# neuraloperator/pde-policylearning

Hardware: AMD Instinct MI355X
Metric: FNO2d fwd+bwd fields/sec (higher is better)
Workload: dtype f32

## Files before the change

### include/fnoengine.h

```cpp
#ifndef FNOENGINE_H
#define FNOENGINE_H
#include <stddef.h>
#ifdef __cplusplus
extern "C" {
#endif

#define FNO_MAX_LAYERS 16
#define FNO_VERSION 100

enum { FNO_OK = 0, FNO_EINVAL = -1, FNO_EUNSUPPORTED = -2, FNO_EHIP = -3, FNO_ENOMEM = -4 };
enum { FNO_NORM_BACKWARD = 0, FNO_NORM_FORWARD = 1, FNO_NORM_ORTHO = 2 };

int fno_version(void);
const char* fno_last_error(void);
void fno_set_gemm_mode(int split_precision);
int fno_get_gemm_mode(void);
void fno_set_mode_gemm(int mfma);
int fno_get_mode_gemm(void);

void fno_set_fused_mid(int on);
int fno_get_fused_mid(void);

typedef struct FnoSpecDesc {
  int ndim;
  int Cin, Cout;
  int dims[3];
  int modes[3];
  int weight_last_extent;
  int norm;
  int input_gelu;
  int weight_planes;
} FnoSpecDesc;

typedef struct FnoSpecPlan FnoSpecPlan;
int fno_spec_plan_create(const FnoSpecDesc* desc, FnoSpecPlan** out);
void fno_spec_plan_destroy(FnoSpecPlan* plan);
size_t fno_spec_workspace_bytes(const FnoSpecPlan* plan, int batch);
size_t fno_spec_xhat_bytes(const FnoSpecPlan* plan, int batch);
int fno_spec_forward(const FnoSpecPlan* plan, int batch, const float* x, const float* const* w_corners,
                     const float* bias , float* y, float* xhat_save, void* ws, size_t ws_bytes,
                     void* stream);
int fno_spec_backward(const FnoSpecPlan* plan, int batch, const float* dy, const float* xhat_save,
                      const float* const* w_corners, float* dx, float* const* dw_corners, float* dbias, void* ws,
                      size_t ws_bytes, void* stream);

typedef struct FnoModelDesc {
  int ndim;
  int Cin, C, Cout;
  int hidden_proj;
  int n_layers;
  int dims[3];
  int modes[3];
  int norm;
  unsigned gelu_mask;
// ... 284 lines not shown
```

### pde_policylearning_amd/csrc/fno_abi.hip

```cpp
#include <hip/hip_runtime.h>

#include <cmath>
#include <cstdarg>
#include <cstdio>
#include <cstdlib>
#include <cstring>
#include <map>
#include <mutex>
#include <string>
#include <vector>

#include "../../include/fnoengine.h"
#include "fno_debug.h"
#include "k_block_bwd.h"
#include "k_block_bwd2.h"
#include "k_chanflow.h"
#include "k_chanflow_step.h"
#include "k_control_loop.h"
#include "k_action_opt.h"
#include "k_policy_opt.h"
#include "k_ns2d.h"
#include "k_pointwise.h"
#include "k_block_fwd2.h"
#include "k_block_fwd3.h"
// ... 388 lines not shown
  }
  if (rc != FNO_AXIS_GENERIC) return rc;
  if (n_out > 65535) return fail(FNO_EUNSUPPORTED, "axis pass grid too large (%d)", n_out);
  return LV(truncating ? "k_axis_generic(truncating)" : "k_axis_generic(extending)", 0, 0), launch("k_axis_generic", k_axis_generic, dim3((inner + 255) / 256, n_out, outer), dim3(256), 0, st, in, out,
                tw, n_in, n_out, inner, truncating ? 1 : 0);
}

static int lead_forward(hipStream_t st, const Geom& g, const Tables& t, bool grad_dir, int B, int C, const float* x1,
                        float* tmp, float* hat) {
  const float2* tw0 = grad_dir ? t.tw_fwd_si[0] : t.tw_fwd_sf[0];
  if (g.nlead == 1) return axis_pass(st, true, x1, hat, tw0, B, g.dims[0], g.Klead[0], g.Klast * C);
  LAUNCHCHK(axis_pass(st, true, x1, tmp, t.tw_fwd_sf[1], B * g.dims[0], g.dims[1], g.Klead[1], g.Klast * C));
  return axis_pass(st, true, tmp, hat, tw0, B, g.dims[0], g.Klead[0], g.Klead[1] * g.Klast * C);
}
static int lead_inverse(hipStream_t st, const Geom& g, const Tables& t, int B, int C, const float* hat, float* tmp,
                        float* z) {
  if (g.nlead == 1) return axis_pass(st, false, hat, z, t.tw_inv[0], B, g.Klead[0], g.dims[0], g.Klast * C);
  LAUNCHCHK(axis_pass(st, false, hat, tmp, t.tw_inv[0], B, g.Klead[0], g.dims[0], g.Klead[1] * g.Klast * C));
  return axis_pass(st, false, tmp, z, t.tw_inv[1], B * g.dims[0], g.Klead[1], g.dims[1], g.Klast * C);
}

static int g_fused_mid = getenv("FNO_NO_FUSED_MID") ? 0 : 1;
extern "C" void fno_set_fused_mid(int on) { g_fused_mid = on ? 1 : 0; }
extern "C" int fno_get_fused_mid(void) { return g_fused_mid; }
static bool fused_mid_shape_ok(const Geom& g, int C) {
  if (g.nlead != 1 || (C != 32 && C != 64) || (g.Klast * C) % 64 != 0) return false;
  if (g.dims[0] > 512) return false;
  const int nk = g.Klead[0];
  return nk == 4 || nk == 8 || nk == 12 || nk == 16;
}
static bool fused_mid_ok(const Geom& g, int C) { return g_fused_mid && fused_mid_shape_ok(g, C); }
template <int NK>
static int spec_mid_t(hipStream_t st, int C, const float2* x1, float2* hat, const float2* wm, float2* z, const float2* twT,
                      const float2* twi, int n, int inner, int K2, int conj_w, int samples, int Bm, size_t w_ms) {
  const size_t lds = (size_t)10 * NK * 64 * 8;
  const dim3 grid(inner / 64, samples), blk(64, 8);
  if (C == 32) return launch("k_spec_mid", k_spec_mid<NK, 32>, grid, blk, lds, st, x1, hat, wm, z, twT, twi, n, inner, K2, conj_w, Bm, w_ms);
  return launch("k_spec_mid", k_spec_mid<NK, 64>, grid, blk, lds, st, x1, hat, wm, z, twT, twi, n, inner, K2, conj_w, Bm, w_ms);
}
static int spectral_mid_fused(hipStream_t st, const Geom& g, const Tables& t, bool grad_dir, int samples, int C,
                              const float* x1, float* hat, const float* wm, float* z, int conj_w, int Bm = 1 << 30,
                              size_t w_ms = 0) {
  if (samples > 65535) return fail(FNO_EUNSUPPORTED, "spectral middle grid too large (%d)", samples);
  const float2* twT = grad_dir ? t.tw_fwd_si[0] : t.tw_fwd_sf[0];
  const float2 *xx = (const float2*)x1, *ww = (const float2*)wm;
  float2 *hh = (float2*)hat, *zz = (float2*)z;
  const int n = g.dims[0], inner = g.Klast * C;
  switch (g.Klead[0]) {
    case 4: return spec_mid_t<4>(st, C, xx, hh, ww, zz, twT, t.tw_inv[0], n, inner, g.Klast, conj_w, samples, Bm, w_ms / 2);
    case 8: return spec_mid_t<8>(st, C, xx, hh, ww, zz, twT, t.tw_inv[0], n, inner, g.Klast, conj_w, samples, Bm, w_ms / 2);
    case 12: return spec_mid_t<12>(st, C, xx, hh, ww, zz, twT, t.tw_inv[0], n, inner, g.Klast, conj_w, samples, Bm, w_ms / 2);
    case 16: return spec_mid_t<16>(st, C, xx, hh, ww, zz, twT, t.tw_inv[0], n, inner, g.Klast, conj_w, samples, Bm, w_ms / 2);
  }
  return fail(FNO_EUNSUPPORTED, "fused spectral middle: %d kept leading modes", g.Klead[0]);
}

static bool mode_gemm_members_ok(int Cin, int Cout) {
  return g_mode_mfma && Cin == Cout && (Cin == 32 || Cin == 64);
}
static int mode_gemm(hipStream_t st, const float* x, const float* w, float* out, int B, int Ktot, int Cin, int Cout,
                     int conj_w, int nm = 1, size_t x_ms = 0, size_t w_ms = 0, size_t o_ms = 0, int trans_w = 0) {
  if (Cout > 256) return fail(FNO_EUNSUPPORTED, "channels > 256");
  if (trans_w && !mode_gemm_members_ok(Cin, Cout)) return fail(FNO_EUNSUPPORTED, "transposed-weight contraction needs the matrix-core kernels");
  if (g_mode_mfma && nm == 1 && B <= 4 && Cin <= 64 && Cout <= 64 && (long)Ktot * Cin * Cout >= (1L << 21)) {
    const float2 *xx = (const float2*)x, *ww = (const float2*)w;
    float2* oo = (float2*)out;
    if (!trans_w) {
      const dim3 grid((Ktot + 3) / 4), blk(256);
      switch (B) {
        case 1: return LV("k_mode_gemv<1>", 0, 0), launch("k_mode_gemv", k_mode_gemv<1>, grid, blk, 0, st, xx, ww, oo, Ktot, Cin, Cout, conj_w);
        case 2: return LV("k_mode_gemv<2>", 0, 0), launch("k_mode_gemv", k_mode_gemv<2>, grid, blk, 0, st, xx, ww, oo, Ktot, Cin, Cout, conj_w);
        case 3: return LV("k_mode_gemv<3>", 0, 0), launch("k_mode_gemv", k_mode_gemv<3>, grid, blk, 0, st, xx, ww, oo, Ktot, Cin, Cout, conj_w);
        default: return LV("k_mode_gemv<4>", 0, 0), launch("k_mode_gemv", k_mode_gemv<4>, grid, blk, 0, st, xx, ww, oo, Ktot, Cin, Cout, conj_w);
      }
    } else if (conj_w) {
      const dim3 grid(Ktot), blk(256);
      const size_t lds = (size_t)Cout * (Cin + 1) * 8;
      switch (B) {
        case 1: return LV("k_mode_gemv_t<1>", 0, 0), launch("k_mode_gemv_t", k_mode_gemv_t<1>, grid, blk, lds, st, xx, ww, oo, Ktot, Cout, Cin);
        case 2: return LV("k_mode_gemv_t<2>", 0, 0), launch("k_mode_gemv_t", k_mode_gemv_t<2>, grid, blk, lds, st, xx, ww, oo, Ktot, Cout, Cin);
        case 3: return LV("k_mode_gemv_t<3>", 0, 0), launch("k_mode_gemv_t", k_mode_gemv_t<3>, grid, blk, lds, st, xx, ww, oo, Ktot, Cout, Cin);
        default: return LV("k_mode_gemv_t<4>", 0, 0), launch("k_mode_gemv_t", k_mode_gemv_t<4>, grid, blk, lds, st, xx, ww, oo, Ktot, Cout, Cin);
      }
    }
  }
// ... 673 lines not shown
template <typename CP, typename P>
static CP corner_ptrs(const Geom& g, P spec_w, int lo, int hi) {
  CP cp;
  memset(&cp, 0, sizeof(cp));
  for (int l = lo; l <= hi; ++l)
    for (int c = 0; c < (1 << g.nlead); ++c) cp.p[l - lo][c] = (std::remove_reference_t<decltype(cp.p[0][0])>)spec_w[l][c];
  return cp;
}

template <int CIN, int COUT>
static int launch_pw(const FnoModelPlan* p, hipStream_t st, int grid, const PwFwdArgs& a, const char* name) {
  const size_t lds = pw_fwd_lds_bytes(CIN, COUT, p->NPX, a.W, a.K2in, a.NJ, a.z != nullptr, a.x1 != nullptr);
  if (p->NPX == 128)
    return GT(1), launch(name, k_pw_fwd<CIN, COUT, 128>, dim3(grid), dim3((COUT / 32) * 4 * 64), lds, st, a);
  return GT(1), launch(name, k_pw_fwd<CIN, COUT, 256>, dim3(grid), dim3((COUT / 32) * 8 * 64), lds, st, a);
}
static int launch_lift(const FnoModelPlan* p, hipStream_t st, int grid, const PwFwdArgs& a) {
  const int C = p->d.C;
  switch (p->d.Cin * 100 + C) {
    case 132: return launch_pw<1, 32>(p, st, grid, a, "k_pw_fwd_lift");
    case 232: return launch_pw<2, 32>(p, st, grid, a, "k_pw_fwd_lift");
    case 332: return launch_pw<3, 32>(p, st, grid, a, "k_pw_fwd_lift");
    case 432: return launch_pw<4, 32>(p, st, grid, a, "k_pw_fwd_lift");
    case 164: return launch_pw<1, 64>(p, st, grid, a, "k_pw_fwd_lift");
    case 264: return launch_pw<2, 64>(p, st, grid, a, "k_pw_fwd_lift");
    case 364: return launch_pw<3, 64>(p, st, grid, a, "k_pw_fwd_lift");
    case 464: return launch_pw<4, 64>(p, st, grid, a, "k_pw_fwd_lift");
  }
  return fail(FNO_EUNSUPPORTED, "lifting %d -> %d", p->d.Cin, C);
}
static bool lift_fused(const FnoModelPlan* p) {
  return p->d.Cin > 0 && g_gemm_x3 && p->NPX == 128 && !p->loose;
}
template <int C>
static bool blk_fwd_t_ok(const FnoModelPlan* p, const PwFwdArgs& a, size_t* lds) {
  if (p->NPX != 128 || p->loose || !a.x) return false;
  if ((size_t)a.PW * 4 * C >= (size_t)1 << 31) return false;
  if (a.z && a.K2in > 8) return false;
  if (C == 32) return false;
  *lds = blk_fwd_t_lds_bytes(C, a.W, a.K2in, a.NJ, a.z != nullptr, a.x1 != nullptr);
  return *lds + 2048 <= FNO_LDS_MAX;
}
static const int g_bfwd_v2 = getenv("FNO_BFWD_V2") ? 1 : 0;
static const int g_zigzag = getenv("FNO_NO_ZIGZAG") ? 0 : 1;
static bool blk_fwd_s_ok(const FnoModelPlan* p, const PwFwdArgs& a, size_t* lds) {
  if (g_bfwd_v2 || p->NPX != 128 || p->loose || !a.x || !a.u || !a.z || !a.xmax) return false;
  if (a.W != 128 || a.K2in < 1 || a.K2in > 8 || a.relu_out || a.add || (a.lw && a.CL > 4)) return false;
  if (a.x1 && (a.NJ != 1 || a.K2out > 8)) return false;
  if ((size_t)a.PW * 4 * 64 >= (size_t)1 << 31) return false;
  *lds = blk_fwd_s_lds_bytes(a.K2out, a.x1 != nullptr);
  return *lds <= FNO_LDS_MAX;
}
template <bool ACT_IN, bool LIFT>
static int launch_blk_fwd_s(const char* nm, hipStream_t st, dim3 grid, size_t lds, int epi, const PwFwdArgs& a) {
  if (epi == 2) return launch(nm, k_blk_fwd_s<ACT_IN, 2, LIFT>, grid, dim3(256), lds, st, a);
  if (epi == 1) return launch(nm, k_blk_fwd_s<ACT_IN, 1, LIFT>, grid, dim3(256), lds, st, a);
  return launch(nm, k_blk_fwd_s<ACT_IN, 0, LIFT>, grid, dim3(256), lds, st, a);
}
template <int C>
static int launch_block_x3(const FnoModelPlan* p, hipStream_t st, int grid, const PwFwdArgs& a, bool* ub_published = nullptr) {
  bool unused = false;
  bool& published = ub_published ? *ub_published : unused;
  published = false;
  const bool lift_ub = a.lw && a.ubound && a.xmax;
  const char* nm = a.lw ? "k_pw_fwd_block0" : "k_pw_fwd_block";
  size_t lds_t = 0, lds_s = 0;
// ... 146 lines not shown
template <int C>
static int launch_pfwd_c(const FnoModelPlan* p, hipStream_t st, int grid, const ProjFwdArgs& a) {
  return a.CO == 1 ? launch_pfwd_cn<C, 1>(p, st, grid, a) : launch_pfwd_cn<C, PROJ_MAXCO>(p, st, grid, a);
}
template <int C, int NCO>
static int launch_pbwd_cn(const FnoModelPlan* p, hipStream_t st, int grid, const ProjBwdArgs& a) {
  const size_t lds = proj_bwd_lds_bytes(C, kHID, p->NPX, NCO);
  GT(1);
  if (p->NPX == 128) return launch("k_proj_bwd", k_proj_bwd<C, kHID, 128, NCO>, dim3(grid), dim3(512), lds, st, a);
  return launch("k_proj_bwd", k_proj_bwd<C, kHID, 256, NCO>, dim3(grid), dim3(1024), lds, st, a);
}
static bool use_pbwd_t(int C, int CO, int npx) {
  return g_gemm_x3 && (C == 64 || C == 32) && CO == 1 && npx == 128;
}
static int w1_frag_items(int HID, int C) { return (HID / 32) * (C / 16) * 64 + (HID / 32) * 2 * (C / 32) * 64; }
static int pack_w1_x3(hipStream_t st, const float* w1, unsigned short* wa1, unsigned short* wa3, int HID, int C) {
  return launch("k_pack_w1_x3", k_pack_w1_t<3>, dim3((w1_frag_items(HID, C) + 255) / 256), dim3(256), 0, st, w1, wa1, wa3, HID, C,
                (const float*)nullptr);
}
template <int C>
static int launch_pbwd_c(const FnoModelPlan* p, hipStream_t st, int grid, const ProjBwdArgs& a) {
  const size_t lds_t = proj_bwd_t_lds_bytes(C, a);
  if (a.wa1 && use_pbwd_t(C, a.CO, p->NPX)) {
    if (a.amax) return GT(2), launch("k_proj_bwd", k_proj_bwd_t<C, kHID, false, 2>, dim3(grid), dim3(512), lds_t, st, a);
    if (lds_t <= FNO_LDS_MAX) return GT(3), launch("k_proj_bwd", k_proj_bwd_t<C, kHID, false>, dim3(grid), dim3(512), lds_t, st, a);
  }
  return a.CO == 1 ? launch_pbwd_cn<C, 1>(p, st, grid, a) : launch_pbwd_cn<C, PROJ_MAXCO>(p, st, grid, a);
}
static int blk_fwd_grid(const FnoModelPlan* p, int ntiles) {
  return std::min(ntiles, (g_gemm_x3 ? FNO_GRID_PWX : FNO_GRID_PW) * p->ncu);
}

static int spectral_mid_fwd(const FnoModelPlan* p, hipStream_t st, int B, const ModelWs& w, const float* wp,
                            float* hat) {
  const Geom& g = p->g;
  const int C = p->d.C;
  if (fused_mid_ok(g, C)) return spectral_mid_fused(st, g, p->t, false, B, C, w.x1, hat, wp, w.z, 0);
  LAUNCHCHK(lead_forward(st, g, p->t, false, B, C, w.x1, w.tmp, hat));
  LAUNCHCHK(mode_gemm(st, hat, wp, w.ohat, B, g.Ktot, C, C, 0));
  return lead_inverse(st, g, p->t, B, C, w.ohat, w.tmp, w.z);
}
static int spectral_mid_adj(const FnoModelPlan* p, hipStream_t st, const ModelSizes& s, int B, int nm, const float* x1, float* tmp,
                            float* ohat, const float* xhat, float* dwp, const float* wps, const float* wpts, float* hat, float* z) {
  const Geom& g = p->g;
  const int C = p->d.C;
  const bool adj_mfma = mode_gemm_members_ok(C, C);
  const size_t hs = nm > 1 ? s.n_hat : 0, ws = nm > 1 ? s.n_wp : 0;
  LAUNCHCHK(lead_forward(st, g, p->t, true, nm * B, C, x1, tmp, ohat));
  if (dwp) LAUNCHCHK(mode_gemm_dw(st, xhat, ohat, dwp, B, g.Ktot, C, C, nm, 0, hs, ws));
  LAUNCHCHK(mode_gemm(st, ohat, adj_mfma ? wps : wpts, hat, B, g.Ktot, C, C, 1, nm, hs, ws, hs, adj_mfma ? 1 : 0));
  return lead_inverse(st, g, p->t, nm * B, C, hat, tmp, z);
}

static int tail_check(const FnoModelPlan* p, const FnoBlockTail* t, bool backward) {
  if (!t) return FNO_OK;
  const FnoModelDesc& d = p->d;
  if (d.Cin != 0 || d.Cout != 0 || d.n_layers != 1) return fail(FNO_EUNSUPPORTED, "block tail: one-layer block stacks only");
  if (p->NPX != 128 || p->loose || !row_fast_ok(p->g, d.C))
    return fail(FNO_EUNSUPPORTED, "block tail: 32 / 64 channels, rows of 32 / 64 / 128 floats");
  if (t->drop_p < 0.f || t->drop_p >= 1.f) return fail(FNO_EINVAL, "block tail: dropout rate %g outside [0, 1)", (double)t->drop_p);
  if (t->drop_p > 0.f && !t->drop_seed) return fail(FNO_EINVAL, "block tail: dropout needs the two seed words (device pointer)");
  if (backward && t->relu_out && !t->y) return fail(FNO_EINVAL, "block tail: the backward of a ReLU tail needs the forward's output");
  return FNO_OK;
}
static int model_forward_impl(const FnoModelPlan* p, int B, const FnoModelParams* prm, const float* x, float* y,
                              void* saved, void* ws, size_t ws_bytes, void* stream, const FnoBlockTail* tail);
extern "C" int fno_model_forward(const FnoModelPlan* p, int B, const FnoModelParams* prm, const float* x, float* y,
                                 void* saved, void* ws, size_t ws_bytes, void* stream) {
  return model_forward_impl(p, B, prm, x, y, saved, ws, ws_bytes, stream, nullptr);
}
extern "C" int fno_model_forward_tail(const FnoModelPlan* p, int B, const FnoModelParams* prm, const float* x, float* y,
                                      void* saved, void* ws, size_t ws_bytes, void* stream, const FnoBlockTail* tail) {
  if (!tail) return fail(FNO_EINVAL, "fno_model_forward_tail: null tail");
  return model_forward_impl(p, B, prm, x, y, saved, ws, ws_bytes, stream, tail);
}
static int model_forward_impl(const FnoModelPlan* p, int B, const FnoModelParams* prm, const float* x, float* y,
                              void* saved, void* ws, size_t ws_bytes, void* stream, const FnoBlockTail* tail) {
  if (!p || !prm || !x || !y || B < 1) return fail(FNO_EINVAL, "fno_model_forward: bad argument");
  if (!saved) return fail(FNO_EINVAL, "fno_model_forward: `saved` buffer required (fno_model_saved_bytes)");
  LAUNCHCHK(tail_check(p, tail, false));
  hipStream_t st = (hipStream_t)stream;
  const Geom& g = p->g;
  const FnoModelDesc& d = p->d;
  const int C = d.C, L = d.n_layers;
  const ModelSizes s = model_sizes(p, B);
  bool ok;
  ModelWs w = carve_model(p, B, ws, ws_bytes, false, &ok);
  if (!ok) return fail(FNO_ENOMEM, "workspace too small: need %zu, have %zu", w.total, ws_bytes);
  const ModelSaved sv = carve_saved(p, B, saved);
  float* const u = sv.u;
  float* const amax = sv.bounds;
  const bool h2 = g_gemm_x3 && d.Cout > 0 && (size_t)B * g.PW >= ((size_t)1 << 17);
  static_assert(kNAmax == 64, "k_pack_w_tiled clears 64 slots");
  LAUNCHCHK(pack_w_layers(st, g, C, C, corner_ptrs<CornerPtrsL>(g, prm->spec_w, 0, L - 1), L, sv.wps,
                          mode_gemm_members_ok(C, C) && !fused_mid_shape_ok(g, C) ? nullptr : sv.wpts, s.n_wp, h2 ? amax : nullptr));

  const bool has_lift = d.Cin > 0, has_proj = d.Cout > 0;
  bool lift_xmax = false;
  bool u0_bound = false;
  FnoModelPlan::CallState cs;
  cs.B = B;
  PwFwdArgs a;
  if (has_lift) {
    memset(&a, 0, sizeof(a));
    a.x = x; a.w = prm->lift_w; a.bias = prm->lift_b;
    cs.u0_skipped = lift_fused(p);
    a.u = cs.u0_skipped ? nullptr : u; a.x1 = p->loose ? nullptr : w.x1; a.tfwd = p->t.tfwd_f;
    set_tile_geom(a, g, s, 0);
    const size_t lds_lr = ((size_t)2 * g.Klast * (g.W + 4) + (size_t)LR_ROWS * d.Cin * (g.W + 4) + 2) * 4 + (size_t)LR_ROWS * g.Klast * (d.Cin + 1) * 8;
    if (cs.u0_skipped && !p->loose && lds_lr <= 48 * 1024) {
      const int nrows = B * g.P;
      LAUNCHCHK(launch("k_lift_rowdft", k_lift_rowdft, dim3((nrows + LR_ROWS - 1) / LR_ROWS), dim3(256), lds_lr, st, x,
                       prm->lift_w, prm->lift_b, p->t.tfwd_f, (float2*)w.x1, d.Cin, C, g.PW, g.W, g.P, g.Klast, nrows,
                       h2 ? amax + kBndX : nullptr));
      lift_xmax = h2;
    } else
    LAUNCHCHK(launch_lift(p, st, std::min(s.ntiles, FNO_GRID_LIFT * p->ncu), a));
    if (p->loose) LAUNCHCHK(row_forward(st, g, p->t.tfwd_f, p->t.tT[0], p->t.K2P, B, C, u, w.x1));
  } else if (tail && tail->drop_p > 0.f) {
    RowMod mod;
    mod.drop_seed = tail->drop_seed; mod.drop_p = tail->drop_p;
    LAUNCHCHK(row_forward(st, g, p->t.tfwd_f, p->t.tT[0], p->t.K2P, B, C, x, w.x1, 0, &mod));
  } else {
    LAUNCHCHK(row_forward(st, g, p->t.tfwd_f, p->t.tT[0], p->t.K2P, B, C, x, w.x1));
  }

  for (int l = 0; l < L; ++l) {
    if (p->loose && l > 0)
      LAUNCHCHK(row_forward(st, g, p->t.tfwd_f, p->t.tT[0], p->t.K2P, B, C, u + (size_t)l * s.n_act, w.x1,
                            (int)((d.gelu_mask >> (l - 1)) & 1u)));
    LAUNCHCHK(spectral_mid_fwd(p, st, B, w, sv.wps + (size_t)l * s.n_wp, sv.hats + (size_t)l * s.n_hat));
    memset(&a, 0, sizeof(a));
    a.x = (l == 0 && !has_lift) ? x : u + (size_t)l * s.n_act;
    if (l == 0 && has_lift && cs.u0_skipped) { a.x = x; a.lw = prm->lift_w; a.lb = prm->lift_b; a.CL = d.Cin; }
    a.w = prm->skip_w[l];
    a.bias = prm->spec_bias ? prm->spec_bias + (size_t)l * C : nullptr;
    a.z = w.z; a.tinv = p->t.tinv_f;
    a.u = (l == L - 1 && !has_proj) ? y : u + (size_t)(l + 1) * s.n_act;
    a.x1 = (l + 1 < L && !p->loose) ? w.x1 : nullptr;
    a.tfwd = p->t.tfwd_f;
    set_tile_geom(a, g, s, g.Klast);
    a.act_in = (l > 0) && ((d.gelu_mask >> (l - 1)) & 1u);
    a.act_out = (d.gelu_mask >> l) & 1u;
    a.relu_out = tail && tail->relu_out;
    if (h2) {
      a.umax = amax + bnd_u(l + 1);
      if (l == 0) { a.xmax = (a.lw && lift_xmax) ? amax + kBndX : nullptr; a.ubound = amax + bnd_u(0); }
      else a.xmax = amax + bnd_u(l);
    }
    a.rev = g_zigzag ? (l & 1) : 0;
    bool ub = false;
    LAUNCHCHK(launch_block(p, st, blk_fwd_grid(p, s.ntiles), a, &ub));
    if (l == 0) u0_bound = ub;
  }

  if (!has_proj) { p->put_call(saved, cs); return FNO_OK; }
  ProjFwdArgs pa;
  memset(&pa, 0, sizeof(pa));
  pa.x = u + (size_t)L * s.n_act; pa.w1 = prm->proj_w1; pa.b1 = prm->proj_b1; pa.w2 = prm->proj_w2; pa.b2 = prm->proj_b2;
  pa.y = y; pa.PW = g.PW; pa.CO = d.Cout; pa.act_in = (d.gelu_mask >> (L - 1)) & 1u;
  pa.tiles_per_plane = g.PW / 128; pa.ntiles = B * pa.tiles_per_plane;
  pa.xmax = h2 ? amax + bnd_u(L) : nullptr;
  cs.h2_fwd = h2;
  cs.bwd_clean = h2;
// ... 1933 lines not shown
```

### pde_policylearning_amd/csrc/k_pointwise.h

```cpp
#pragma once
#include "fno_dev.h"

static constexpr int FNO_OCC_PW = 4;
static constexpr int FNO_OCC_PWX = 2;

struct PwFwdArgs {
  const float* x;
  const float* w;
  const float* bias;
  const float* z;
  const float* tinv;
  float* u;
  float* x1;
  const float* tfwd;
  const float* add;
  int PW, W, P, K2in, K2out, NJ;
  int act_in, act_out;
  int relu_out;
  int loose;
  const float* lw;
  const float* lb;
  int CL;
  int tiles_per_plane, ntiles;
  const float* xmax;
// ... 340 lines not shown
#pragma unroll
            for (int h8 = 0; h8 < 2; ++h8) {
              float t[8];
#pragma unroll
              for (int j = 0; j < 8; ++j) t[j] = acc[q][8 * h8 + j];
              gelu8(t, six, inf);
#pragma unroll
              for (int j = 0; j < 8; ++j) xp[((j & 3) + 8 * (2 * h8 + (j >> 2))) * PITCH] = t[j];
            }
          } else {
#pragma unroll
            for (int r = 0; r < 16; ++r) xp[((r & 3) + 8 * (r >> 2)) * PITCH] = acc[q][r];
          }
        }
      }
      if (a.umax) absmax_publish(vmax, a.umax);
    }
    FNO_STAMP(tslot + 5);
    if (a.x1) {
      __syncthreads();
      FNO_STAMP(tslot + 6);
      row_dft_epilogue<C, NPX, NW>(xs, tfwd_s, a.W + 4, a.x1, b, px0, a.P, a.W, a.K2out, a.NJ, wave, lane);
    }
    FNO_STAMP(tslot + 7);
    __syncthreads();
    tslot += 8;
  }
}

constexpr int LR_ROWS = 8;
__global__ void __launch_bounds__(256) k_lift_rowdft(const float* __restrict__ x, const float* __restrict__ lw,
                                                     const float* __restrict__ lb, const float* __restrict__ tfwd,
                                                     float2* __restrict__ x1, int CL, int C, int PW, int W, int P, int K2,
                                                     int nrows, float* __restrict__ xmax) {
  extern __shared__ __attribute__((aligned(16))) float smem[];
  const int WP = W + 4;
  float* ts = smem;
  float* xs = ts + 2 * K2 * WP;
  float2* xh = reinterpret_cast<float2*>(xs + ((LR_ROWS * CL * WP + 1) & ~1));
  const int tid = threadIdx.x, lane = tid & 63, wave = tid >> 6;
  const int row0 = blockIdx.x * LR_ROWS;
  const int nr = min(LR_ROWS, nrows - row0);
  float vmax = 0.f;
  const int c = lane;
  float wv[4];
#pragma unroll
  for (int k = 0; k < 4; ++k) wv[k] = (c < C && k < CL) ? lw[c * CL + k] : 0.f;
  const float bc = (lb && c < C) ? lb[c] : 0.f;
  {
    const int nt_tab = 2 * K2 * W, nt_x = LR_ROWS * CL * W;
    for (int base = 0; base < nt_tab; base += 8 * 256) {
      float v[8];
#pragma unroll
      for (int q = 0; q < 8; ++q) { const int i = base + q * 256 + tid; v[q] = i < nt_tab ? tfwd[i] : 0.f; }
#pragma unroll
      for (int q = 0; q < 8; ++q) { const int i = base + q * 256 + tid; if (i < nt_tab) ts[(i / W) * WP + i % W] = v[q]; }
    }
    for (int base = 0; base < nt_x; base += 8 * 256) {
      float v[8];
#pragma unroll
      for (int q = 0; q < 8; ++q) {
        const int i = base + q * 256 + tid;
        const int rk = i / W, w = i - rk * W, r = rk / CL, k = rk - r * CL;
        const int row = row0 + r;
        const int b = row / P, prow = row - b * P;
        v[q] = (i < nt_x && r < nr) ? x[((size_t)b * CL + k) * PW + (size_t)prow * W + w] : 0.f;
      }
#pragma unroll
      for (int q = 0; q < 8; ++q) {
        const int i = base + q * 256 + tid;
        if (i < nt_x) { xs[(i / W) * WP + i % W] = v[q]; vmax = fmaxf(vmax, fabsf(v[q])); }
      }
    }
  }
  if (xmax) {
#pragma unroll
    for (int o = 32; o >= 1; o >>= 1) vmax = fmaxf(vmax, __shfl_xor(vmax, o, 64));
    __shared__ float wmax[4];
    if (lane == 0) wmax[wave] = vmax;
    __syncthreads();
    vmax = fmaxf(fmaxf(wmax[0], wmax[1]), fmaxf(wmax[2], wmax[3]));
    if (wave == 0 && (blockIdx.x & 15) == 0) absmax_publish(vmax, xmax);
  }
  __syncthreads();
  for (int i = tid; i < LR_ROWS * K2 * (CL + 1); i += 256) {
    const int r = i / (K2 * (CL + 1)), k2 = (i / (CL + 1)) % K2, k = i % (CL + 1);
    const float* tr = ts + (2 * k2) * WP;
    const float* ti = tr + WP;
    float sr = 0.f, si = 0.f;
    if (k < CL) {
      const float* xr = xs + (r * CL + k) * WP;
      float sr2 = 0.f, si2 = 0.f;
#pragma unroll 4
      for (int w = 0; w < W; w += 4) {
        const float4 xv = *reinterpret_cast<const float4*>(xr + w), tv = *reinterpret_cast<const float4*>(tr + w),
                     uv = *reinterpret_cast<const float4*>(ti + w);
        sr = fmaf(xv.x, tv.x, sr); si = fmaf(xv.x, uv.x, si);
        sr2 = fmaf(xv.y, tv.y, sr2); si2 = fmaf(xv.y, uv.y, si2);
        sr = fmaf(xv.z, tv.z, sr); si = fmaf(xv.z, uv.z, si);
        sr2 = fmaf(xv.w, tv.w, sr2); si2 = fmaf(xv.w, uv.w, si2);
      }
      sr += sr2; si += si2;
    } else {
      for (int w = 0; w < W; ++w) { sr += tr[w]; si += ti[w]; }
    }
    xh[i] = make_float2(sr, si);
  }
  __syncthreads();
  if (c < C) {
    float2* dst = x1 + (size_t)row0 * K2 * C + c;
    for (int p = wave; p < nr * K2; p += 4) {
      const float2* h = xh + p * (CL + 1);
      float sr = bc * h[CL].x, si = bc * h[CL].y;
#pragma unroll
      for (int k = 0; k < 4; ++k)
        if (k < CL) { sr = fmaf(wv[k], h[k].x, sr); si = fmaf(wv[k], h[k].y, si); }
      dst[(size_t)p * C] = make_float2(sr, si);
    }
  }
  if (xmax && wave == 0 && (blockIdx.x & 15) != 0) absmax_publish(vmax, xmax);
}
```

### pde_policylearning_amd/csrc/k_spectral_mid.h

```cpp
#pragma once
#include "fno_dev.h"

template <int NR, int SEGS = 8, bool TLDS = false>
__global__ void __launch_bounds__(64 * SEGS) k_axis_fwd(const float2* __restrict__ in, float2* __restrict__ out,
                                                        const float2* __restrict__ twT_g, int n_in, int inner) {
  extern __shared__ __attribute__((aligned(16))) float smem[];
  float2* sh = reinterpret_cast<float2*>(smem);
  const int ql = threadIdx.x;
  const int seg = __builtin_amdgcn_readfirstlane(threadIdx.y);
  const int q = blockIdx.x * 64 + ql;
  const int o = blockIdx.y;
  const float2* twT = twT_g;
  if constexpr (TLDS) {
    for (int i = threadIdx.y * 64 + threadIdx.x; i < n_in * NR; i += 64 * SEGS) sh[i] = twT_g[i];
    __syncthreads();
    twT = sh;
  }
  float2 acc[NR];
#pragma unroll
  for (int r = 0; r < NR; ++r) acc[r] = make_float2(0.f, 0.f);
  if (q < inner) {
    const float2* src = in + (size_t)o * n_in * inner + q;
    for (int nb = seg; nb < n_in; nb += 8 * SEGS) {
      float2 v[8];
// ... 978 lines not shown
      const size_t b = e / PW, p = e % PW;
      s += dy[(b * C + c) * PW + p];
    }
  }
  for (int off = 32; off > 0; off >>= 1) s += __shfl_xor(s, off, 64);
  __shared__ float sh[4];
  if ((threadIdx.x & 63) == 0) sh[threadIdx.x >> 6] = s;
  __syncthreads();
  if (threadIdx.x == 0) part[(size_t)blockIdx.x * C + c] = sh[0] + sh[1] + sh[2] + sh[3];
}

#ifdef FNO_TRACE
#define MID_STAMP(slot) do { if (blockIdx.x == 2 && blockIdx.y == gridDim.y / 2 && threadIdx.x == 0) \
    g_trace[threadIdx.y * 256 + (slot)] = __builtin_readcyclecounter(); \
    if (blockIdx.x == 0 && threadIdx.x == 0 && threadIdx.y == 0 && ((slot) == 0 || (slot) == 7)) \
    g_trace[8 * 256 + blockIdx.y * 2 + ((slot) == 7)] = __builtin_readcyclecounter(); \
    if (blockIdx.x == 1 && threadIdx.x == 0 && threadIdx.y == 0 && blockIdx.y < 64)  \
    g_trace[10 * 256 + blockIdx.y * 8 + (slot)] = __builtin_readcyclecounter(); } while (0)
#else
#define MID_STAMP(slot) do { } while (0)
#endif
template <bool B> struct MidFlag { static constexpr bool value = B; };
template <bool SREG>
FNO_DEV void cfma_uniform(f32x2& acc, float2 w, f32x2 v, f32x2 vs) {
  if constexpr (SREG) {
    const f32x2 wp = {w.x, w.y};
    asm("v_pk_fma_f32 %0, %1, %2, %0 op_sel_hi:[0,1,1]" : "+v"(acc) : "s"(wp), "v"(v));
    asm("v_pk_fma_f32 %0, %1, %2, %0 op_sel:[1,0,0] op_sel_hi:[1,1,1]" : "+v"(acc) : "s"(wp), "v"(vs));
  } else {
    acc[0] = fmaf(w.x, v[0], acc[0]); acc[0] = fmaf(w.y, vs[0], acc[0]);
    acc[1] = fmaf(w.x, v[1], acc[1]); acc[1] = fmaf(w.y, vs[1], acc[1]);
  }
}
template <int NK, int C>
__global__ void __launch_bounds__(512, 4) k_spec_mid(const float2* __restrict__ x1, float2* __restrict__ hat,
                                                     const float2* __restrict__ wm, float2* __restrict__ z,
                                                     const float2* __restrict__ twT, const float2* __restrict__ twi, int n,
                                                     int inner, int K2, int conj_w, int Bm, size_t w_ms) {
  static_assert(C == 32 || C == 64, "whole bins per workgroup");
  constexpr bool SREG = NK <= 12;
  constexpr int SEGS = 8, JW = C / SEGS, NTH = 64 * SEGS;
  constexpr int RB = 2, NG = NK / RB;
  static_assert(NK % RB == 0, "mode groups");
  extern __shared__ __attribute__((aligned(16))) float smem[];
  float2* sh = reinterpret_cast<float2*>(smem);
  float2* ys = sh + SEGS * NK * 64;
  float2* os = ys + NK * 64;
  const int ql = threadIdx.x;
  const int seg = __builtin_amdgcn_readfirstlane(threadIdx.y);
  const int tid = seg * 64 + ql;
  const int q = blockIdx.x * 64 + ql;
  const int o = blockIdx.y;
  const int k2 = q / C, ch = q - k2 * C, lb = (ql / C) * C;
  const float2* wb = wm + (size_t)(o / Bm) * w_ms + ((size_t)k2 * C + seg * JW) * C + ch;
  MID_STAMP(0);
  if constexpr (!SREG) for (int i = tid; i < n * NK; i += NTH) sh[i] = twT[i];
  float2 wv[2][RB][JW];
  auto load_w = [&](int g, int buf) {
#pragma unroll
    for (int rr = 0; rr < RB; ++rr)
#pragma unroll
      for (int j = 0; j < JW; ++j) wv[buf][rr][j] = wb[((size_t)(g * RB + rr) * K2 * C + j) * C];
  };
  load_w(0, 0);
  {
    f32x2 acc[NK];
#pragma unroll
    for (int r = 0; r < NK; ++r) acc[r] = f32x2{0.f, 0.f};
    const float2* src = x1 + (size_t)o * n * inner + q;
    constexpr int NBR = 16;
    bool first = true;
    for (int nb = seg; nb < n; nb += NBR * SEGS) {
      float2 v[NBR];
#pragma unroll
      for (int j = 0; j < NBR; ++j) {
        const int nn = nb + SEGS * j;
        v[j] = nn < n ? src[(size_t)nn * inner] : make_float2(0.f, 0.f);
      }
      if constexpr (SREG) {
      (void)first;
      auto rows = [&](auto guard) {
        constexpr bool GUARD = decltype(guard)::value;
        float2 tw[2][NK];
#pragma unroll
        for (int r = 0; r < NK; ++r) tw[0][r] = twT[(size_t)min(nb, n - 1) * NK + r];
#pragma unroll
        for (int j = 0; j < NBR; ++j) {
          const int nn = nb + SEGS * j;
          if (j + 1 < NBR) {
#pragma unroll
            for (int r = 0; r < NK; ++r) tw[(j + 1) & 1][r] = twT[(size_t)(GUARD ? min(nn + SEGS, n - 1) : nn + SEGS) * NK + r];
          }
          if (!GUARD || nn < n) {
            const f32x2 vv = {v[j].x, v[j].y}, vs = natural_pair(-v[j].y, v[j].x);
#pragma unroll
            for (int r = 0; r < NK; ++r) cfma_uniform<true>(acc[r], tw[j & 1][r], vv, vs);
          }
        }
      };
      if (nb + SEGS * (NBR - 1) < n) rows(MidFlag<false>{}); else rows(MidFlag<true>{});
      } else {
      if (first) { __syncthreads(); first = false; }
#pragma unroll
      for (int j = 0; j < NBR; ++j) {
        const int nn = nb + SEGS * j;
        if (nn < n) {
          const float2* t = sh + nn * NK;
          const f32x2 vv = {v[j].x, v[j].y}, vs = natural_pair(-v[j].y, v[j].x);
#pragma unroll
          for (int r = 0; r < NK; ++r) cfma_uniform<false>(acc[r], t[r], vv, vs);
        }
      }
      }
    }
    if constexpr (!SREG) { if (first) __syncthreads(); }
    MID_STAMP(1);
    if constexpr (!SREG) __syncthreads();
#pragma unroll
    for (int r = 0; r < NK; ++r) sh[(seg * NK + r) * 64 + ql] = make_float2(acc[r][0], acc[r][1]);
  }
  __syncthreads();
  MID_STAMP(2);
  for (int r = seg; r < NK; r += SEGS) {
    float sx = 0.f, sy = 0.f;
#pragma unroll
    for (int k = 0; k < SEGS; ++k) { sx += sh[(k * NK + r) * 64 + ql].x; sy += sh[(k * NK + r) * 64 + ql].y; }
    ys[r * 64 + ql] = make_float2(sx, sy);
    if (hat) hat[((size_t)o * NK + r) * inner + q] = make_float2(sx, sy);
  }
  __syncthreads();
  MID_STAMP(3);
  {
    const float sg = conj_w ? -1.f : 1.f;
#pragma unroll
    for (int g = 0; g < NG; ++g) {
      if (g + 1 < NG) load_w(g + 1, (g + 1) & 1);
#pragma unroll
      for (int rr = 0; rr < RB; ++rr) {
        float ax = 0.f, ay = 0.f;
#pragma unroll
        for (int j = 0; j < JW; ++j) {
          const float2 y = ys[(g * RB + rr) * 64 + lb + seg * JW + j];
          const float2 w = wv[g & 1][rr][j];
          const float wy = sg * w.y;
          ax = fmaf(y.x, w.x, ax); ax = fmaf(-y.y, wy, ax);
          ay = fmaf(y.x, wy, ay); ay = fmaf(y.y, w.x, ay);
        }
        sh[(seg * NK + g * RB + rr) * 64 + ql] = make_float2(ax, ay);
      }
    }
  }
  MID_STAMP(4);
  __syncthreads();
  MID_STAMP(5);
  for (int r = seg; r < NK; r += SEGS) {
    float sx = 0.f, sy = 0.f;
#pragma unroll
    for (int k = 0; k < SEGS; ++k) { sx += sh[(k * NK + r) * 64 + ql].x; sy += sh[(k * NK + r) * 64 + ql].y; }
    os[r * 64 + ql] = make_float2(sx, sy);
  }
  __syncthreads();
// ... 53 lines not shown
```

Measured before the change: 30190.

## Apply lifting in mode space so first spectral layer reads raw-channel row spectra

When the lift is fused with the row DFT, the row-DFT kernel now writes row spectra of the few raw input channels (plus a constant-row spectrum for the bias) rather than of the full lifted C-channel field. The first-layer spectral middle kernel gets a LIFTIN variant that runs the column DFT on these narrow spectra and applies the linear lift and bias in mode space before the channel mixing. Because the DFT is linear, this cuts the first layer's x1 write and read from C channels down to at most four. It adds a kernel specialisation with its own lane layout that relies on the mode and channel limits holding.

```diff
diff --git a/include/fnoengine.h b/include/fnoengine.h
--- a/include/fnoengine.h
+++ b/include/fnoengine.h
@@ -20,6 +20,8 @@
 
 void fno_set_fused_mid(int on);
 int fno_get_fused_mid(void);
+void fno_set_lift_modespace(int on);
+int fno_get_lift_modespace(void);
 
 typedef struct FnoSpecDesc {
   int ndim;
diff --git a/pde_policylearning_amd/csrc/fno_abi.hip b/pde_policylearning_amd/csrc/fno_abi.hip
--- a/pde_policylearning_amd/csrc/fno_abi.hip
+++ b/pde_policylearning_amd/csrc/fno_abi.hip
@@ -444,25 +444,32 @@
 static bool fused_mid_ok(const Geom& g, int C) { return g_fused_mid && fused_mid_shape_ok(g, C); }
 template <int NK>
 static int spec_mid_t(hipStream_t st, int C, const float2* x1, float2* hat, const float2* wm, float2* z, const float2* twT,
-                      const float2* twi, int n, int inner, int K2, int conj_w, int samples, int Bm, size_t w_ms) {
+                      const float2* twi, int n, int inner, int K2, int conj_w, int samples, int Bm, size_t w_ms,
+                      const MidLiftIn* lift) {
   const size_t lds = (size_t)10 * NK * 64 * 8;
   const dim3 grid(inner / 64, samples), blk(64, 8);
-  if (C == 32) return launch("k_spec_mid", k_spec_mid<NK, 32>, grid, blk, lds, st, x1, hat, wm, z, twT, twi, n, inner, K2, conj_w, Bm, w_ms);
-  return launch("k_spec_mid", k_spec_mid<NK, 64>, grid, blk, lds, st, x1, hat, wm, z, twT, twi, n, inner, K2, conj_w, Bm, w_ms);
+  MidLiftIn li;
+  memset(&li, 0, sizeof(li));
+  if (lift) {
+    if (C != 64 || lift->CL < 1 || lift->CL > 4) return fail(FNO_EUNSUPPORTED, "lifting-input spectral middle: %d -> %d channels", lift->CL, C);
+    return LV("k_spec_mid<LIFTIN>", 0, 0), launch("k_spec_mid", k_spec_mid<NK, 64, true>, grid, blk, lds, st, x1, hat, wm, z, twT, twi, n, inner, K2, conj_w, Bm, w_ms, *lift);
+  }
+  if (C == 32) return launch("k_spec_mid", k_spec_mid<NK, 32>, grid, blk, lds, st, x1, hat, wm, z, twT, twi, n, inner, K2, conj_w, Bm, w_ms, li);
+  return launch("k_spec_mid", k_spec_mid<NK, 64>, grid, blk, lds, st, x1, hat, wm, z, twT, twi, n, inner, K2, conj_w, Bm, w_ms, li);
 }
 static int spectral_mid_fused(hipStream_t st, const Geom& g, const Tables& t, bool grad_dir, int samples, int C,
                               const float* x1, float* hat, const float* wm, float* z, int conj_w, int Bm = 1 << 30,
-                              size_t w_ms = 0) {
+                              size_t w_ms = 0, const MidLiftIn* lift = nullptr) {
   if (samples > 65535) return fail(FNO_EUNSUPPORTED, "spectral middle grid too large (%d)", samples);
   const float2* twT = grad_dir ? t.tw_fwd_si[0] : t.tw_fwd_sf[0];
   const float2 *xx = (const float2*)x1, *ww = (const float2*)wm;
   float2 *hh = (float2*)hat, *zz = (float2*)z;
   const int n = g.dims[0], inner = g.Klast * C;
   switch (g.Klead[0]) {
-    case 4: return spec_mid_t<4>(st, C, xx, hh, ww, zz, twT, t.tw_inv[0], n, inner, g.Klast, conj_w, samples, Bm, w_ms / 2);
-    case 8: return spec_mid_t<8>(st, C, xx, hh, ww, zz, twT, t.tw_inv[0], n, inner, g.Klast, conj_w, samples, Bm, w_ms / 2);
-    case 12: return spec_mid_t<12>(st, C, xx, hh, ww, zz, twT, t.tw_inv[0], n, inner, g.Klast, conj_w, samples, Bm, w_ms / 2);
-    case 16: return spec_mid_t<16>(st, C, xx, hh, ww, zz, twT, t.tw_inv[0], n, inner, g.Klast, conj_w, samples, Bm, w_ms / 2);
+    case 4: return spec_mid_t<4>(st, C, xx, hh, ww, zz, twT, t.tw_inv[0], n, inner, g.Klast, conj_w, samples, Bm, w_ms / 2, lift);
+    case 8: return spec_mid_t<8>(st, C, xx, hh, ww, zz, twT, t.tw_inv[0], n, inner, g.Klast, conj_w, samples, Bm, w_ms / 2, lift);
+    case 12: return spec_mid_t<12>(st, C, xx, hh, ww, zz, twT, t.tw_inv[0], n, inner, g.Klast, conj_w, samples, Bm, w_ms / 2, lift);
+    case 16: return spec_mid_t<16>(st, C, xx, hh, ww, zz, twT, t.tw_inv[0], n, inner, g.Klast, conj_w, samples, Bm, w_ms / 2, lift);
   }
   return fail(FNO_EUNSUPPORTED, "fused spectral middle: %d kept leading modes", g.Klead[0]);
 }
@@ -1202,6 +1209,17 @@
 static bool lift_fused(const FnoModelPlan* p) {
   return p->d.Cin > 0 && g_gemm_x3 && p->NPX == 128 && !p->loose;
 }
+static size_t lift_rowdft_lds(const FnoModelPlan* p) {
+  const Geom& g = p->g;
+  return ((size_t)2 * g.Klast * (g.W + 4) + (size_t)LR_ROWS * p->d.Cin * (g.W + 4) + 2) * 4 + (size_t)LR_ROWS * g.Klast * (p->d.Cin + 1) * 8;
+}
+static int g_lift_modespace = 1;
+extern "C" void fno_set_lift_modespace(int on) { g_lift_modespace = on ? 1 : 0; }
+extern "C" int fno_get_lift_modespace(void) { return g_lift_modespace; }
+static bool lift_modespace(const FnoModelPlan* p) {
+  return g_lift_modespace && lift_fused(p) && lift_rowdft_lds(p) <= 48 * 1024 && fused_mid_ok(p->g, p->d.C) && p->d.C == 64 &&
+         p->d.Cin <= 4;
+}
 template <int C>
 static bool blk_fwd_t_ok(const FnoModelPlan* p, const PwFwdArgs& a, size_t* lds) {
   if (p->NPX != 128 || p->loose || !a.x) return false;
@@ -1414,10 +1432,11 @@
 }
 
 static int spectral_mid_fwd(const FnoModelPlan* p, hipStream_t st, int B, const ModelWs& w, const float* wp,
-                            float* hat) {
+                            float* hat, const MidLiftIn* lift = nullptr) {
   const Geom& g = p->g;
   const int C = p->d.C;
-  if (fused_mid_ok(g, C)) return spectral_mid_fused(st, g, p->t, false, B, C, w.x1, hat, wp, w.z, 0);
+  if (fused_mid_ok(g, C)) return spectral_mid_fused(st, g, p->t, false, B, C, w.x1, hat, wp, w.z, 0, 1 << 30, 0, lift);
+  if (lift) return fail(FNO_EUNSUPPORTED, "lifting-input spectra without the one-launch middle");
   LAUNCHCHK(lead_forward(st, g, p->t, false, B, C, w.x1, w.tmp, hat));
   LAUNCHCHK(mode_gemm(st, hat, wp, w.ohat, B, g.Ktot, C, C, 0));
   return lead_inverse(st, g, p->t, B, C, w.ohat, w.tmp, w.z);
@@ -1483,18 +1502,24 @@
   FnoModelPlan::CallState cs;
   cs.B = B;
   PwFwdArgs a;
+  MidLiftIn mli;
+  memset(&mli, 0, sizeof(mli));
   if (has_lift) {
     memset(&a, 0, sizeof(a));
     a.x = x; a.w = prm->lift_w; a.bias = prm->lift_b;
     cs.u0_skipped = lift_fused(p);
     a.u = cs.u0_skipped ? nullptr : u; a.x1 = p->loose ? nullptr : w.x1; a.tfwd = p->t.tfwd_f;
     set_tile_geom(a, g, s, 0);
-    const size_t lds_lr = ((size_t)2 * g.Klast * (g.W + 4) + (size_t)LR_ROWS * d.Cin * (g.W + 4) + 2) * 4 + (size_t)LR_ROWS * g.Klast * (d.Cin + 1) * 8;
+    const size_t lds_lr = lift_rowdft_lds(p);
     if (cs.u0_skipped && !p->loose && lds_lr <= 48 * 1024) {
       const int nrows = B * g.P;
+      if (lift_modespace(p)) {
+        mli.xl = (const float2*)w.x1; mli.srow = mli.xl + (size_t)nrows * g.Klast * d.Cin;
+        mli.lw = prm->lift_w; mli.lb = prm->lift_b; mli.CL = d.Cin;
+      }
       LAUNCHCHK(launch("k_lift_rowdft", k_lift_rowdft, dim3((nrows + LR_ROWS - 1) / LR_ROWS), dim3(256), lds_lr, st, x,
                        prm->lift_w, prm->lift_b, p->t.tfwd_f, (float2*)w.x1, d.Cin, C, g.PW, g.W, g.P, g.Klast, nrows,
-                       h2 ? amax + kBndX : nullptr));
+                       h2 ? amax + kBndX : nullptr, (float2*)mli.xl, (float2*)mli.srow));
       lift_xmax = h2;
     } else
     LAUNCHCHK(launch_lift(p, st, std::min(s.ntiles, FNO_GRID_LIFT * p->ncu), a));
@@ -1511,7 +1536,8 @@
     if (p->loose && l > 0)
       LAUNCHCHK(row_forward(st, g, p->t.tfwd_f, p->t.tT[0], p->t.K2P, B, C, u + (size_t)l * s.n_act, w.x1,
                             (int)((d.gelu_mask >> (l - 1)) & 1u)));
-    LAUNCHCHK(spectral_mid_fwd(p, st, B, w, sv.wps + (size_t)l * s.n_wp, sv.hats + (size_t)l * s.n_hat));
+    LAUNCHCHK(spectral_mid_fwd(p, st, B, w, sv.wps + (size_t)l * s.n_wp, sv.hats + (size_t)l * s.n_hat,
+                               (l == 0 && mli.xl) ? &mli : nullptr));
     memset(&a, 0, sizeof(a));
     a.x = (l == 0 && !has_lift) ? x : u + (size_t)l * s.n_act;
     if (l == 0 && has_lift && cs.u0_skipped) { a.x = x; a.lw = prm->lift_w; a.lb = prm->lift_b; a.CL = d.Cin; }
diff --git a/pde_policylearning_amd/csrc/k_pointwise.h b/pde_policylearning_amd/csrc/k_pointwise.h
--- a/pde_policylearning_amd/csrc/k_pointwise.h
+++ b/pde_policylearning_amd/csrc/k_pointwise.h
@@ -396,7 +396,8 @@
 __global__ void __launch_bounds__(256) k_lift_rowdft(const float* __restrict__ x, const float* __restrict__ lw,
                                                      const float* __restrict__ lb, const float* __restrict__ tfwd,
                                                      float2* __restrict__ x1, int CL, int C, int PW, int W, int P, int K2,
-                                                     int nrows, float* __restrict__ xmax) {
+                                                     int nrows, float* __restrict__ xmax, float2* __restrict__ xl,
+                                                     float2* __restrict__ srow) {
   extern __shared__ __attribute__((aligned(16))) float smem[];
   const int WP = W + 4;
   float* ts = smem;
@@ -409,8 +410,8 @@
   const int c = lane;
   float wv[4];
 #pragma unroll
-  for (int k = 0; k < 4; ++k) wv[k] = (c < C && k < CL) ? lw[c * CL + k] : 0.f;
-  const float bc = (lb && c < C) ? lb[c] : 0.f;
+  for (int k = 0; k < 4; ++k) wv[k] = (!xl && c < C && k < CL) ? lw[c * CL + k] : 0.f;
+  const float bc = (!xl && lb && c < C) ? lb[c] : 0.f;
   {
     const int nt_tab = 2 * K2 * W, nt_x = LR_ROWS * CL * W;
     for (int base = 0; base < nt_tab; base += 8 * 256) {
@@ -468,7 +469,15 @@
     } else {
       for (int w = 0; w < W; ++w) { sr += tr[w]; si += ti[w]; }
     }
+    if (xl) {
+      if (k < CL) { if (r < nr) xl[((size_t)(row0 + r) * K2 + k2) * CL + k] = make_float2(sr, si); }
+      else if (row0 == 0 && r == 0) srow[k2] = make_float2(sr, si);
+    } else
     xh[i] = make_float2(sr, si);
+  }
+  if (xl) {
+    if (xmax && wave == 0 && (blockIdx.x & 15) != 0) absmax_publish(vmax, xmax);
+    return;
   }
   __syncthreads();
   if (c < C) {
diff --git a/pde_policylearning_amd/csrc/k_spectral_mid.h b/pde_policylearning_amd/csrc/k_spectral_mid.h
--- a/pde_policylearning_amd/csrc/k_spectral_mid.h
+++ b/pde_policylearning_amd/csrc/k_spectral_mid.h
@@ -1034,12 +1034,20 @@
     acc[1] = fmaf(w.x, v[1], acc[1]); acc[1] = fmaf(w.y, vs[1], acc[1]);
   }
 }
-template <int NK, int C>
+struct MidLiftIn {
+  const float2* xl;
+  const float2* srow;
+  const float* lw;
+  const float* lb;
+  int CL;
+};
+template <int NK, int C, bool LIFTIN = false>
 __global__ void __launch_bounds__(512, 4) k_spec_mid(const float2* __restrict__ x1, float2* __restrict__ hat,
                                                      const float2* __restrict__ wm, float2* __restrict__ z,
                                                      const float2* __restrict__ twT, const float2* __restrict__ twi, int n,
-                                                     int inner, int K2, int conj_w, int Bm, size_t w_ms) {
+                                                     int inner, int K2, int conj_w, int Bm, size_t w_ms, MidLiftIn li) {
   static_assert(C == 32 || C == 64, "whole bins per workgroup");
+  static_assert(!LIFTIN || (C == 64 && NK * 4 <= 64), "lifting input: one bin per workgroup, a lane per (mode, input channel)");
   constexpr bool SREG = NK <= 12;
   constexpr int SEGS = 8, JW = C / SEGS, NTH = 64 * SEGS;
   constexpr int RB = 2, NG = NK / RB;
@@ -1056,7 +1064,7 @@
   const int k2 = q / C, ch = q - k2 * C, lb = (ql / C) * C;
   const float2* wb = wm + (size_t)(o / Bm) * w_ms + ((size_t)k2 * C + seg * JW) * C + ch;
   MID_STAMP(0);
-  if constexpr (!SREG) for (int i = tid; i < n * NK; i += NTH) sh[i] = twT[i];
+  if constexpr (!SREG && !LIFTIN) for (int i = tid; i < n * NK; i += NTH) sh[i] = twT[i];
   float2 wv[2][RB][JW];
   auto load_w = [&](int g, int buf) {
 #pragma unroll
@@ -1065,6 +1073,57 @@
       for (int j = 0; j < JW; ++j) wv[buf][rr][j] = wb[((size_t)(g * RB + rr) * K2 * C + j) * C];
   };
   load_w(0, 0);
+  if constexpr (LIFTIN) {
+    constexpr int NBR = 16;
+    const int CL = li.CL;
+    const int r = ql >> 2, k = ql & 3;
+    const bool live = r < NK && k < CL;
+    const float wl[4] = {CL > 0 ? li.lw[ql * CL] : 0.f, CL > 1 ? li.lw[ql * CL + 1] : 0.f, CL > 2 ? li.lw[ql * CL + 2] : 0.f,
+                         CL > 3 ? li.lw[ql * CL + 3] : 0.f};
+    const float bc = li.lb ? li.lb[ql] : 0.f;
+    const float2 sk = li.srow[k2];
+    float ax = 0.f, ay = 0.f, tx = 0.f, ty = 0.f;
+    const float2* src = li.xl + ((size_t)o * n * K2 + k2) * CL + (live ? k : 0);
+    const float2* tws = twT + (r < NK ? r : 0);
+    for (int nb = seg; nb < n; nb += NBR * SEGS) {
+      float2 v[NBR], t[NBR];
+#pragma unroll
+      for (int j = 0; j < NBR; ++j) {
+        const int nn = nb + SEGS * j;
+        const bool in = nn < n;
+        v[j] = (in && live) ? src[(size_t)nn * K2 * CL] : make_float2(0.f, 0.f);
+        t[j] = in ? tws[(size_t)nn * NK] : make_float2(0.f, 0.f);
+      }
+#pragma unroll
+      for (int j = 0; j < NBR; ++j) {
+        ax = fmaf(t[j].x, v[j].x, ax); ax = fmaf(-t[j].y, v[j].y, ax);
+        ay = fmaf(t[j].x, v[j].y, ay); ay = fmaf(t[j].y, v[j].x, ay);
+        tx += t[j].x; ty += t[j].y;
+      }
+    }
+    MID_STAMP(1);
+    if (r < NK) {
+      sh[(seg * NK + r) * 5 + k] = make_float2(ax, ay);
+      if (k == 0) sh[(seg * NK + r) * 5 + 4] = make_float2(tx, ty);
+    }
+    __syncthreads();
+    MID_STAMP(2);
+    for (int rr = seg; rr < NK; rr += SEGS) {
+      float2 xh[5];
+#pragma unroll
+      for (int kk = 0; kk < 5; ++kk) {
+        float sx = 0.f, sy = 0.f;
+#pragma unroll
+        for (int s8 = 0; s8 < SEGS; ++s8) { sx += sh[(s8 * NK + rr) * 5 + kk].x; sy += sh[(s8 * NK + rr) * 5 + kk].y; }
+        xh[kk] = make_float2(sx, sy);
+      }
+      float sx = bc * (sk.x * xh[4].x - sk.y * xh[4].y), sy = bc * (sk.x * xh[4].y + sk.y * xh[4].x);
+#pragma unroll
+      for (int kk = 0; kk < 4; ++kk) { sx = fmaf(wl[kk], xh[kk].x, sx); sy = fmaf(wl[kk], xh[kk].y, sy); }
+      ys[rr * 64 + ql] = make_float2(sx, sy);
+      if (hat) hat[((size_t)o * NK + rr) * inner + q] = make_float2(sx, sy);
+    }
+  } else {
   {
     f32x2 acc[NK];
 #pragma unroll
@@ -1129,6 +1188,7 @@
     for (int k = 0; k < SEGS; ++k) { sx += sh[(k * NK + r) * 64 + ql].x; sy += sh[(k * NK + r) * 64 + ql].y; }
     ys[r * 64 + ql] = make_float2(sx, sy);
     if (hat) hat[((size_t)o * NK + r) * inner + q] = make_float2(sx, sy);
+  }
   }
   __syncthreads();
   MID_STAMP(3);
```

Result: no change. 30490, median of 4 (+1.0%).
